# second-state/qwen3_asr_rs

Measured on AMD Instinct MI355X. Metric: audio-seconds/sec (RTFx) Qwen3-ASR-0.6B greedy, 30s clips, higher is better.
Workload: dtype bf16; 1 GPU; Qwen3-ASR-0.6b bf16, batch=1 x 30s synthetic 16kHz clip per GPU, 100 new tokens (fixed, EOS ignored); clips_per_gpu=1, parallelism=dp1 (independent utterances per GPU, no data-path collective)

## Files before the change

### qwen3_asr_rs_amd/csrc/dev.h

```cpp
#pragma once
#include <hip/hip_runtime.h>
#include <stdint.h>

#ifdef Q3A_STAMP
#define Q3A_STAMP_FIELD unsigned long long* stamp = nullptr;
#define Q3A_STAMP_AT(ptr, wg, slot) do { if ((ptr) && threadIdx.x == 0) (ptr)[(size_t)(wg) * 8 + (slot)] = wall_clock64(); } while (0)
#else
#define Q3A_STAMP_FIELD
#define Q3A_STAMP_AT(ptr, wg, slot) do { } while (0)
#endif

#define Q3A_ARG(x) asm volatile("" ::"s"(x))

namespace q3a {

typedef __attribute__((ext_vector_type(8))) __bf16 bf16x8_t;
typedef __attribute__((ext_vector_type(4))) float f32x4_t;
typedef __attribute__((ext_vector_type(2))) float f32x2_t;
typedef __attribute__((ext_vector_type(16))) float f32x16_t;

__device__ __forceinline__ float bf16_bits_to_f32(uint32_t v) { return __uint_as_float(v << 16); }
typedef __attribute__((ext_vector_type(2))) __bf16 bf16x2_t;
__device__ __forceinline__ uint32_t pack_bf16x2(float lo, float hi) {
  const f32x2_t v = {lo, hi};
// ... 105 lines not shown

__device__ __forceinline__ float lane_bcast(float v, int lane_uniform) {
  return __int_as_float(__builtin_amdgcn_readlane(__float_as_int(v), lane_uniform));
}

__device__ __forceinline__ float own_vgpr(float x) {
  asm volatile("" : "+v"(x));
  return x;
}
__device__ __forceinline__ void rope_rotate(float n1, float n2, float c, float sn, float& x1, float& x2) {
  const float a = sn * n2, b = sn * n1;
  x1 = __builtin_fmaf(c, n1, -a);
  x2 = __builtin_fmaf(c, n2, b);
}

__device__ __forceinline__ void head_norm_rope(float& x1, float& x2, const float* __restrict__ w, float eps,
                                               const float* __restrict__ cos_t, const float* __restrict__ sin_t,
                                               int pos, int lane) {
  const float ss = wave_sum_fast(x1 * x1 + x2 * x2);
  const float rstd = 1.0f / sqrtf(ss / 128.0f + eps);
  const float c = cos_t[(size_t)pos * 64 + lane], sn = sin_t[(size_t)pos * 64 + lane];
  const float n1 = (x1 * rstd) * w[lane], n2 = (x2 * rstd) * w[lane + 64];
  rope_rotate(n1, n2, c, sn, x1, x2);
}

template <typename T> struct KvIo;
template <> struct KvIo<float> {
  static __device__ __forceinline__ float load(const float* p) { return *p; }
  static __device__ __forceinline__ void store(float* p, float v) { *p = v; }
  static __device__ __forceinline__ float round(float v) { return v; }
};
template <> struct KvIo<uint16_t> {
  static __device__ __forceinline__ float load(const uint16_t* p) { return bf16_bits_to_f32(*p); }
  static __device__ __forceinline__ void store(uint16_t* p, float v) { *p = (uint16_t)f32_to_bf16_bits(v); }
  static __device__ __forceinline__ float round(float v) { return bf16_bits_to_f32(f32_to_bf16_bits(v)); }
};

}
// ... 1 lines not shown
```

### qwen3_asr_rs_amd/csrc/engine.cpp

```cpp
#include <hip/hip_runtime.h>

#include <sched.h>

#include <algorithm>
#include <atomic>
#include <chrono>
#include <cmath>
#include <cstdio>
#include <cstring>
#include <map>
#include <memory>
#include <mutex>
#include <string>
#include <thread>
#include <vector>

#include "../../include/q3asr.h"
#include "kernels.h"
#include "model.h"

using namespace q3a;

namespace {

// ... 77 lines not shown
}
namespace q3a {
struct KnobEntry { const char* key; const char* env; std::atomic<int> Knobs::*field; };
static const KnobEntry kKnobTable[] = {
    {"gemm256_min_tiles", "Q3A_GEMM256_MIN_TILES", &Knobs::gemm256_min_tiles},
    {"gemm256_persist", "Q3A_GEMM256_PERSIST", &Knobs::gemm256_persist},
    {"gemm256_group_m", "Q3A_GEMM256_GROUP_M", &Knobs::gemm256_group_m},
    {"dattn_batched_min_wgs", "Q3A_DATTN_BATCHED_MIN_WGS", &Knobs::dattn_batched_min_wgs},
    {"decode_group_size", "Q3A_DECODE_GROUP", &Knobs::decode_group_size},
    {"decode_parallel_groups", "Q3A_DECODE_PARALLEL", &Knobs::decode_parallel_groups},
    {"fuse_qkrope", "Q3A_FUSE_QKROPE", &Knobs::fuse_qkrope},
    {"skinny_q", "Q3A_SKINNY_Q", &Knobs::skinny_q},
    {"eos_run_ahead", "Q3A_EOS_RUN_AHEAD", &Knobs::eos_run_ahead},
    {"skinny_glu_hp3", "Q3A_SKINNY_GLU_HP3", &Knobs::skinny_glu_hp3},
    {"lm_head_prune", "Q3A_LM_HEAD_PRUNE", &Knobs::lm_head_prune},
    {"layer_taps", "Q3A_DEBUG_LAYER_TAPS", &Knobs::layer_taps},
    {"poison_attn_partials", nullptr, &Knobs::poison_attn_partials},
};
Knobs& knobs() {
  static Knobs k;
  static std::once_flag once;
  std::call_once(once, [] {
    for (const KnobEntry& t : kKnobTable)
      if (const char* e = t.env ? getenv(t.env) : nullptr) (k.*t.field).store(atoi(e));
  });
  return k;
}
}

struct q3a_engine {
// ... 693 lines not shown
  void run_prefill_layers() {
    const int H = d.hidden, I = d.inter, QD = d.q_dim(), QKV = d.qkv_dim();
    const bool sp = precise();
    KCHK(launch_embed(ids.as<int>(), total_P, wh(L.embed), H, kAudioPad, dec_x.as<float>(), stream));
    scatter_audio_rows();
    tap("dec_embed", dec_x.p, (size_t)total_P * H * 4);
    AttnArgs at{};
    at.q = dec_qkv.as<float>(); at.q_rs = QKV; at.kv_hs = (int64_t)max_ctx * 128; at.kv_rs = 128;
    at.o = dec_ctx.as<float>(); at.o_rs = QD; at.segs = dec_segs.as<AttnSeg>(); at.n_segs = B;
    at.max_len = *std::max_element(P.begin(), P.end()); at.n_kv_heads = d.n_kv;
    at.scale_div = sqrtf((float)d.head_dim);
    at.o16 = valu_attn() ? nullptr : dec_ctx.as<uint16_t>();
    if (!valu_attn()) { at.q16 = dec_q16.as<uint16_t>(); at.q_rs = QD; }
    const DevBuf& ctx_in = (valu_attn() && !sp) ? dec_ctx16 : dec_ctx;
    const bool qkv_bias = arena_flags & kFlagDecQkvBias, o_bias = arena_flags & kFlagDecOBias, mlp_bias = arena_flags & kFlagDecMlpBias;
    const bool fuse_rope = knobs().fuse_qkrope.load() != 0 && !valu_attn() && !precise() && d.head_dim == 128 && gemm256_eligible(total_P, QKV, H) && H % 64 == 0;
    const bool layer_taps = opts.debug_taps && knobs().layer_taps.load() != 0;
    for (int li = 0; li < d.dec_layers; ++li) {
      const DecLayerOff& l = L.dec[li];
      auto ltap = [&](const char* what, const void* ptr, size_t bytes) {
        if (!layer_taps) return;
        char name[32];
        snprintf(name, sizeof(name), "L%02d_%s", li, what);
        tap(name, ptr, bytes);
      };
      KCHK(launch_rmsnorm(dec_x.as<float>(), wf(l.in_ln), dec_ln.as<float>(), total_P, H, d.rms_eps, stream, act16(dec_ln)));
      ltap("ln1", dec_ln.p, (size_t)total_P * H * act_elem());
      RopeKvArgs rk{};
      rk.qkv = dec_qkv.as<float>(); rk.row_seq = row_seq.as<int>(); rk.row_pos = row_pos.as<int>();
      rk.q_norm = wf(l.q_norm); rk.k_norm = wf(l.k_norm); rk.eps = d.rms_eps;
      rk.cos_t = rope_cos.as<float>(); rk.sin_t = rope_sin.as<float>();
      rk.kcache = kc_layer(li); rk.vcache = vc_layer(li); rk.n_q = d.n_q; rk.n_kv = d.n_kv; rk.max_ctx = max_ctx;
      rk.q16 = valu_attn() ? nullptr : dec_q16.as<uint16_t>();
      if (fuse_rope) {
        KCHK(launch_gemm256_qkrope(dec_ln.as<uint16_t>(), H, wh(l.qkv_w), total_P, H, qkv_bias ? wf(l.qkv_b) : nullptr, rk, stream));
      } else {
        GemmEpilogue ep; ep.out = dec_qkv.as<float>(); ep.ldo = QKV; ep.bias = qkv_bias ? wf(l.qkv_b) : nullptr;
        act_gemm(dec_ln, H, wh(l.qkv_w), total_P, QKV, H, ep, false);
        KCHK(launch_qknorm_rope_kv(rk, total_P, kv_f32(), stream));
      }
      at.k = kc_layer(li); at.v = vc_layer(li);
      if (fuse_rope) {
        ltap("qkvs", dec_qkv.p, std::min((size_t)1024, (size_t)total_P) * QKV * 4);
      }
      if (!valu_attn()) ltap("q", dec_q16.p, (size_t)total_P * QD * 2);
      ltap("k", kc_layer(li), (size_t)B * d.n_kv * max_ctx * 128 * kv_elem());
      ltap("v", vc_layer(li), (size_t)B * d.n_kv * max_ctx * 128 * kv_elem());
      if (valu_attn()) {
        KCHK(launch_attn_prefill(at, d.n_q / d.n_kv, kv_f32(), stream));
        if (!sp) KCHK(launch_to_bf16(dec_ctx.as<float>(), dec_ctx16.as<uint16_t>(), (size_t)total_P * QD, stream));
// ... 1522 lines not shown
```

### qwen3_asr_rs_amd/csrc/k_fattn.hip

```cpp
#include <stdlib.h>

#include "dev.h"
#include "kernels.h"

namespace q3a {
namespace {

#ifndef Q3A_FATTN_XCD_REMAP
#define Q3A_FATTN_XCD_REMAP 1
#endif
__device__ __forceinline__ void fattn_block(int& bx, int& by, int& bz) {
  bx = blockIdx.x; by = blockIdx.y; bz = blockIdx.z;
#if Q3A_FATTN_XCD_REMAP
  const int gx = gridDim.x, gy = gridDim.y, total = gx * gy * (int)gridDim.z;
  const int lin = bx + gx * (by + gy * bz);
  const int xcd = lin & 7, loc = lin >> 3, q = total >> 3, r = total & 7;
  const int id = (xcd < r ? xcd * (q + 1) : r * (q + 1) + (xcd - r) * q) + loc;
  bx = id % gx;
  const int t = id / gx;
  by = t % gy;
  bz = t / gy;
#endif
}

// ... 421 lines not shown
      for (int r4 = 0; r4 < 4; ++r4) {
        const int d = dt * 32 + 8 * r4 + 4 * half;
        const float4 v = make_float4(oacc[dt][4 * r4] * inv, oacc[dt][4 * r4 + 1] * inv, oacc[dt][4 * r4 + 2] * inv, oacc[dt][4 * r4 + 3] * inv);
        if (a.o16) {
          uint2 pk;
          pk.x = pack_bf16x2(v.x, v.y);
          pk.y = pack_bf16x2(v.z, v.w);
          *reinterpret_cast<uint2*>(a.o16 + (size_t)(seg.q_row0 + qi) * a.o_rs + head * HD + d) = pk;
        } else {
          *reinterpret_cast<float4*>(orow + d) = v;
        }
      }
  }
}

template <int HD, int GROUP, bool CAUSAL>
void launch_dma(const AttnArgs& a, hipStream_t s) {
  constexpr int QT = 32 * (4 / GROUP);
  dim3 grid((a.max_len + QT - 1) / QT, a.n_kv_heads, a.n_segs);
  static const int ns = [] { const char* e = getenv("Q3A_FATTN_NS"); return e ? atoi(e) : 3; }();
  if (ns == 4) hipLaunchKernelGGL((fattn_dma_kernel<HD, GROUP, CAUSAL, 4>), grid, dim3(256), 0, s, a);
  else hipLaunchKernelGGL((fattn_dma_kernel<HD, GROUP, CAUSAL, 3>), grid, dim3(256), 0, s, a);
}
static bool fattn_dma_on() {
  static const bool on = [] { const char* e = getenv("Q3A_FATTN_DMA"); return !e || atoi(e) != 0; }();
  return on;
}

static bool fattn_dma_ok(const AttnArgs& a) {
  const auto al16 = [](const void* p) { return (reinterpret_cast<uintptr_t>(p) & 15) == 0; };
// ... 18 lines not shown
    else launch_f<64, 1, false, uint16_t>(a, s);
  } else {
    launch_f<64, 1, false, float>(a, s);
  }
  return nullptr;
}

const char* launch_fattn_prefill(const AttnArgs& a, int group, hipStream_t s) {
  if (a.n_segs <= 0) return nullptr;
  if (a.q_rs % 4 != 0 || a.o_rs % 4 != 0) return "fattn: row strides must be multiples of 4";
  if (a.q16 && a.q_rs % 8 != 0) return "fattn: bf16 q row stride must be a multiple of 8";
  static const int ks_wgs = [] { const char* e = getenv("Q3A_FATTN_KSPLIT_MAX_WGS"); return e ? atoi(e) : 128; }();
  const long wgs64 = (long)((a.max_len + 63) / 64) * a.n_kv_heads * a.n_segs;
  const bool dma = fattn_dma_ok(a);
  if (group == 1) { if (dma) launch_dma<128, 1, true>(a, s); else launch_f<128, 1, true, uint16_t>(a, s); }
  else if (group == 2 && wgs64 < ks_wgs) launch_f<128, 2, true, uint16_t, 2>(a, s);
  else if (group == 2) { if (dma) launch_dma<128, 2, true>(a, s); else launch_f<128, 2, true, uint16_t>(a, s); }
  else if (group == 4) { if (dma) launch_dma<128, 4, true>(a, s); else launch_f<128, 4, true, uint16_t>(a, s); }
  else return "fattn: GQA group must be 1, 2 or 4";
  return nullptr;
}

}
```

### qwen3_asr_rs_amd/csrc/k_gemm16.hip

```cpp
#include <stdlib.h>

#include <type_traits>

#include "argmax.h"

namespace q3a {
namespace {

typedef const void __attribute__((address_space(1)))* gptr_t;
typedef void __attribute__((address_space(3)))* lptr_t;

struct DenseA16 {
  const uint16_t* x;
  int lda;
  __device__ __forceinline__ void init_row(int m, int M, int& s0, int& s1, int& s2) const {
    s0 = m < M ? m : M - 1;
    s1 = s2 = 0;
  }
  __device__ __forceinline__ const uint16_t* row_ptr(int s0, int, int, int k0) const { return x + (size_t)s0 * lda + k0; }
};

struct ConvA16 {
  const uint16_t* x;
  const uint16_t* zero;
// ... 9 lines not shown
    const int tap = k0 / C, c0 = k0 - tap * C;
    const int kh = tap / 3, kw = tap - kh * 3;
    const int ih = oh * 2 - 1 + kh, iw = ow * 2 - 1 + kw;
    if (ih < 0 || ih >= H || iw < 0 || iw >= W) return zero;
    return x + (((size_t)img * H + ih) * W + iw) * C + c0;
  }
};

template <int BK> __device__ __forceinline__ int swz(int row) { return BK == 64 ? (row >> 1) & 7 : (row >> 2) & 3; }

template <int N> __device__ __forceinline__ void g16_wait_vm() {
  static_assert(N >= 0 && N < 64, "vmcnt value");
  asm volatile("s_waitcnt vmcnt(%0)" ::"n"(N) : "memory");
}

template <int BM, int BN, int BK, bool GLU, class ALoader, int NS = 2, bool LP = false>
__global__ __launch_bounds__(256) void gemm16_kernel(ALoader A, const uint16_t* __restrict__ Wt, int M, int N, int K,
                                                     GemmEpilogue ep) {
  constexpr int CPR = BK / 8;
  constexpr int RPI = 64 / CPR;
  constexpr int A_LOADS = BM / (4 * RPI) > 0 ? BM / (4 * RPI) : 1;
  constexpr int W_LOADS = BN / (4 * RPI) > 0 ? BN / (4 * RPI) : 1;
  constexpr bool A_PART = BM < 4 * RPI, W_PART = BN < 4 * RPI;
  constexpr int MI = BM / 32, NI = BN / 32;
  static_assert(MI >= 1 && NI >= 1 && (!GLU || NI >= 2), "tile shape");
  static_assert(NS == 2 || ((NS == 3 || NS == 4) && !A_PART && !W_PART), "stage count");
  constexpr int STAGE = (BM + BN) * BK;
  __shared__ __attribute__((aligned(16))) uint16_t lds[NS * STAGE];
  Q3A_STAMP_AT(ep.stamp, blockIdx.x, 0);

  const int tiles_m = (M + BM - 1) / BM, tiles_n = (N + BN - 1) / BN;
  const int nwg = tiles_m * tiles_n;
  int bid = blockIdx.x;
  {
    const int q = nwg / 8, r = nwg % 8, xcd = bid % 8, loc = bid / 8;
    bid = (xcd < r ? xcd * (q + 1) : r * (q + 1) + (xcd - r) * q) + loc;
  }
  const int tm = bid % tiles_m, tn = bid / tiles_m;
  const int m0 = tm * BM, n0 = tn * BN;
  const int tid = threadIdx.x, lane = tid & 63, wave = tid >> 6;
  const int wr = wave >> 1, wc = wave & 1;

  const int l_row = lane / CPR, l_chunk = lane % CPR;
  const bool a_on = !A_PART || wave * RPI < BM, w_on = !W_PART || wave * RPI < BN;
  int a_s0[A_LOADS], a_s1[A_LOADS], a_s2[A_LOADS], a_src_chunk[A_LOADS];
  const uint16_t* w_src[W_LOADS];
#pragma unroll
  for (int i = 0; i < A_LOADS; ++i) {
    const int row = (i * 4 + wave) * RPI + l_row;
    a_src_chunk[i] = l_chunk ^ swz<BK>(row);
    A.init_row(m0 + row, M, a_s0[i], a_s1[i], a_s2[i]);
  }
#pragma unroll
  for (int i = 0; i < W_LOADS; ++i) {
    const int row = (i * 4 + wave) * RPI + l_row;
    const int n = n0 + row;
    w_src[i] = Wt + (size_t)(n < N ? n : N - 1) * K + (l_chunk ^ swz<BK>(row)) * 8;
// ... 29 lines not shown
      for (int i = 0; i < MI; ++i) {
        const int mc = mrow[i] < M ? mrow[i] : M - 1;
#pragma unroll
        for (int j = 0; j < NI; ++j) ad[i][j] = *reinterpret_cast<const float4*>(ep.addend + (size_t)(mc % ep.addend_period) * ep.ldo + ncl[j]);
      }
    }
    if (ep.resid) {
#pragma unroll
      for (int i = 0; i < MI; ++i) {
        const int oc = orow[i] < 0 ? 0 : orow[i];
#pragma unroll
        for (int j = 0; j < NI; ++j) rs[i][j] = *reinterpret_cast<const float4*>(ep.resid + (size_t)oc * ep.ldo + ncl[j]);
      }
    }
  };
  const bool pre = !GLU && MI * NI <= 4 && vec && ep.rowmap == nullptr;
  if (pre) load_operands();

  const int frag_row = lane & 15, frag_kc = lane >> 4;
  const int KT = K / BK;
  auto issue_tile = [&](int kt, int buf) {
    const int k0 = kt * BK;
    if (a_on) {
#pragma unroll
      for (int i = 0; i < A_LOADS; ++i) {
        const int base = (i * 4 + wave) * RPI * BK;
        const uint16_t* ap = A.row_ptr(a_s0[i], a_s1[i], a_s2[i], k0) + a_src_chunk[i] * 8;
        __builtin_amdgcn_global_load_lds((gptr_t)ap, (lptr_t)(lds + buf * STAGE + base), 16, 0, 0);
      }
    }
    if (w_on) {
#pragma unroll
// ... 34 lines not shown
      for (int j = 0; j < NI; ++j) {
        const int row = wc * (BN / 2) + j * 16 + frag_row;
        bfrag[j] = *reinterpret_cast<const bf16x8_t*>(&ws[row * BK + (((ks * 4 + frag_kc) ^ swz<BK>(row)) * 8)]);
      }
#pragma unroll
      for (int i = 0; i < MI; ++i) {
        const int row = wr * (BM / 2) + i * 16 + frag_row;
        const bf16x8_t af = *reinterpret_cast<const bf16x8_t*>(&as[row * BK + (((ks * 4 + frag_kc) ^ swz<BK>(row)) * 8)]);
#pragma unroll
        for (int j = 0; j < NI; ++j) acc[i][j] = __builtin_amdgcn_mfma_f32_16x16x32_bf16(bfrag[j], af, acc[i][j], 0, 0, 0);
      }
    }
  }

  Q3A_STAMP_AT(ep.stamp, blockIdx.x, 2);
  if (ep.rowmap) {
#pragma unroll
    for (int i = 0; i < MI; ++i) orow[i] = ep.rowmap[orow[i]];
  }
  if (!GLU && vec) {
    if (!pre) load_operands();
    constexpr bool ARGMAX = BM == 32 && MI == 1;
    static_assert(!LP || ARGMAX, "the log-sum channel rides on the argmax partials");
    ArgmaxAcc<LP> best;
    float lv[LP ? NI : 1][4];
    if constexpr (LP) {
#pragma unroll
      for (int j = 0; j < NI; ++j) lv[j][0] = lv[j][1] = lv[j][2] = lv[j][3] = -INFINITY;
    }
#pragma unroll
// ... 350 lines not shown
  if (n == 0) return nullptr;
  size_t blocks = (n + 255) / 256;
  if (blocks > 4096) blocks = 4096;
  hipLaunchKernelGGL(from_bf16_kernel, dim3((unsigned)blocks), dim3(256), 0, s, x, y, n);
  return nullptr;
}

const char* launch_gemm16(const uint16_t* X, int lda, const uint16_t* W, int M, int N, int K, const GemmEpilogue& ep,
                          bool glu, hipStream_t s) {
  if (M <= 0) return nullptr;
  if (K % 32 != 0 || lda % 8 != 0) return "gemm16: K must be a multiple of 32 and lda of 8";
  if (K % 64 == 0 && !ep.part.val && gemm256_eligible(M, N, K)) return launch_gemm256(X, lda, W, M, N, K, ep, glu, s);
  return launch_gemm16_small(X, lda, W, M, N, K, ep, glu, s);
}

const char* launch_gemm16_small(const uint16_t* X, int lda, const uint16_t* W, int M, int N, int K, const GemmEpilogue& ep,
                                bool glu, hipStream_t s) {
  if (M <= 0) return nullptr;
  if (K % 32 != 0 || lda % 8 != 0) return "gemm16: K must be a multiple of 32 and lda of 8";
  if (glu && N % 32 != 0) return "gemm16: GLU needs N % 32 == 0";
  if (const char* e = argmax_partials_check(ep.part, (N + 63) / 64)) return e;
  if (ep.part.val && (M > 32 || glu || N % 4 != 0 || ep.ldo % 4 != 0 || K % 64 != 0 || ep.rowmap))
    return "gemm16: argmax partials need M <= 32, 4 | N, 4 | ldo, 64 | K and no row map";
  DenseA16 A{X, lda};
  static const bool ksplit_on = [] { const char* e = getenv("Q3A_GEMM16_KSPLIT"); return !e || atoi(e) != 0; }();
  if (ksplit_on && !glu && !ep.part.val && tiles_of(M, N, 32, 64) < 384 && K >= 512 && K % 128 == 0 && N % 4 == 0 && ep.ldo % 4 == 0) {
    const int tiles = ((M + 31) / 32) * ((N + 31) / 32);
    if (K % 256 == 0) hipLaunchKernelGGL((gemm16k_kernel<32, 256, DenseA16, 2>), dim3(tiles), dim3(256), 0, s, A, W, M, N, K, ep);
    else hipLaunchKernelGGL((gemm16k_kernel<32, 128, DenseA16, 4>), dim3(tiles), dim3(256), 0, s, A, W, M, N, K, ep);
    return nullptr;
  }
  static const bool force_bk32 = [] { const char* e = getenv("Q3A_GEMM16_BK32"); return e && atoi(e) != 0; }();
  if (K % 64 == 0 && !force_bk32) {
    if (glu) launch_sized16<64, true>(A, W, M, N, K, ep, s); else launch_sized16<64, false>(A, W, M, N, K, ep, s);
  } else {
    if (glu) launch_sized16<32, true>(A, W, M, N, K, ep, s); else launch_sized16<32, false>(A, W, M, N, K, ep, s);
  }
  return nullptr;
}

const char* launch_to_bf16(const float* x, uint16_t* y, size_t n, hipStream_t s) {
  if (n == 0) return nullptr;
  if (n % 4 != 0) return "to_bf16: n must be a multiple of 4";
  size_t blocks = (n / 4 + 255) / 256;
  if (blocks > 4096) blocks = 4096;
  hipLaunchKernelGGL(to_bf16_kernel, dim3((unsigned)blocks), dim3(256), 0, s, x, y, n / 4);
  return nullptr;
}

const char* launch_conv3x3s2_gemm16(const uint16_t* X, const uint16_t* zero_page, int imgs, int H, int Wd, int C,
                                    const uint16_t* Wt, int Cout, const GemmEpilogue& ep, hipStream_t s) {
  if (C % 32 != 0) return "conv gemm16: C must be a multiple of 32";
// ... 11 lines not shown
```

### qwen3_asr_rs_amd/csrc/k_mel.hip

```cpp
#include "dev.h"
#include "kernels.h"

namespace q3a {
namespace {

constexpr int N_FFT = 400, HOP = 160, N_FREQ = 201, DFT_COLS = 416, N_MELS = 128;
constexpr int FRAMES_PER_BLOCK = 32;
constexpr int SAMPLES_PER_BLOCK = (FRAMES_PER_BLOCK - 1) * HOP + N_FFT;
constexpr int P_STRIDE = 209;
constexpr int K_MEL = 202;

__device__ __forceinline__ unsigned float_key(float x) {
  unsigned u = __float_as_uint(x);
  return (u & 0x80000000u) ? ~u : (u | 0x80000000u);
}
__device__ __forceinline__ float key_float(unsigned k) {
  return __uint_as_float((k & 0x80000000u) ? (k & 0x7fffffffu) : ~k);
}

__global__ __launch_bounds__(256) void mel_kernel(MelBatch mb, const float* __restrict__ dft,
                                                  const float* __restrict__ filt_t) {
  __shared__ float s_lds[SAMPLES_PER_BLOCK + SAMPLES_PER_BLOCK / HOP + 8];
  __shared__ float p_lds[FRAMES_PER_BLOCK * P_STRIDE];
  const int b = blockIdx.y;
  const int F = mb.n_frames[b];
  const int f0 = blockIdx.x * FRAMES_PER_BLOCK;
  if (f0 >= F) return;
  const int64_t n = mb.n_samples[b];
  const int64_t Lp = (int64_t)F * HOP;
  const float* pcm = mb.pcm + mb.pcm_off[b];
  const int tid = threadIdx.x, lane = tid & 63, wave = tid >> 6, half = lane >> 5, l31 = lane & 31;

  for (int p = tid; p < SAMPLES_PER_BLOCK; p += 256) {
    int64_t i = (int64_t)f0 * HOP + p - N_FFT / 2;
    if (i < 0) i = -i;
    else if (i >= Lp) i = 2 * (Lp - 1) - i;
    float v = 0.f;
    if (i >= 0 && i < n) v = pcm[i];
    s_lds[p + p / HOP] = v;
  }
  for (int i = tid; i < FRAMES_PER_BLOCK * P_STRIDE; i += 256) p_lds[i] = 0.f;
  __syncthreads();

  const int a_base = l31 * (HOP + 1);
  for (int tile = wave; tile < DFT_COLS / 32; tile += 4) {
    f32x16_t acc;
#pragma unroll
    for (int r = 0; r < 16; ++r) acc[r] = 0.f;
    const float* bcol = dft + tile * 32 + l31;
#pragma unroll 4
    for (int nn = 0; nn < N_FFT; nn += 2) {
      const int m = nn + half;
      const float a = s_lds[a_base + m + (m >= HOP) + (m >= 2 * HOP)];
      const float bv = bcol[(size_t)m * DFT_COLS];
      acc = __builtin_amdgcn_mfma_f32_32x32x2f32(a, bv, acc, 0, 0, 0);
    }
    const int c = tile * 32 + l31, k = c >> 1;
#pragma unroll
    for (int r = 0; r < 16; ++r) {
      float pw = acc[r] * acc[r];
      pw += __shfl_xor(pw, 1, 64);
      const int frame = (r & 3) + 8 * (r >> 2) + 4 * half;
      if ((c & 1) == 0 && k < P_STRIDE - 1) p_lds[frame * P_STRIDE + k] = pw;
    }
  }
  __syncthreads();

  f32x16_t acc;
#pragma unroll
  for (int r = 0; r < 16; ++r) acc[r] = 0.f;
  const float* acol = filt_t + wave * 32 + l31;
  const float* brow = p_lds + l31 * P_STRIDE;
#pragma unroll 4
  for (int kk = 0; kk < K_MEL; kk += 2) {
    const int k = kk + half;
    acc = __builtin_amdgcn_mfma_f32_32x32x2f32(acol[(size_t)k * N_MELS], brow[k], acc, 0, 0, 0);
  }
  const int f = f0 + l31;
  float vmax = -3.0e38f;
  float* out = mb.mel + mb.mel_off[b];
#pragma unroll
  for (int r = 0; r < 16; ++r) {
    const int m = wave * 32 + (r & 3) + 8 * (r >> 2) + 4 * half;
    const float lv = log10f(fmaxf(acc[r], 1e-10f));
    if (f < F) {
      out[(size_t)m * F + f] = lv;
      vmax = fmaxf(vmax, lv);
    }
  }
  vmax = wave_max(vmax);
  if (lane == 0) atomicMax(mb.gmax_key + b, float_key(vmax));
// ... 4 lines not shown
  const int64_t total = (int64_t)mb.n_frames[b] * N_MELS;
  const float floor_v = key_float(mb.gmax_key[b]) - 8.0f;
  float* m = mb.mel + mb.mel_off[b];
  for (int64_t i = (int64_t)blockIdx.x * blockDim.x + threadIdx.x; i < total; i += (int64_t)gridDim.x * blockDim.x)
    m[i] = (fmaxf(m[i], floor_v) + 4.0f) / 4.0f;
}

}

const char* launch_mel(const MelBatch& mb, int B, int max_frames, const float* dft, const float* filt_t,
                       hipStream_t s) {
  if (B <= 0) return nullptr;
  hipError_t e = hipMemsetAsync(mb.gmax_key, 0, sizeof(unsigned) * B, s);
  if (e != hipSuccess) return "mel: memset failed";
  const int tiles = (max_frames + FRAMES_PER_BLOCK - 1) / FRAMES_PER_BLOCK;
  hipLaunchKernelGGL(mel_kernel, dim3(tiles, B), dim3(256), 0, s, mb, dft, filt_t);
  int fb = (max_frames * N_MELS + 255) / 256;
  if (fb > 1024) fb = 1024;
  hipLaunchKernelGGL(mel_finalize_kernel, dim3(fb, B), dim3(256), 0, s, mb);
  return nullptr;
}

}
```

### qwen3_asr_rs_amd/csrc/kernels.h

```cpp
#pragma once
#include <hip/hip_runtime.h>
#include <stdint.h>

#include <atomic>

#ifndef Q3A_STAMP_FIELD
#ifdef Q3A_STAMP
#define Q3A_STAMP_FIELD unsigned long long* stamp = nullptr;
#else
#define Q3A_STAMP_FIELD
#endif
#endif

namespace q3a {

struct ArgmaxPartials {
  float* val = nullptr;
  int* idx = nullptr;
  float* sum = nullptr;
  int stride = 0;
  ArgmaxPartials at(size_t rows) const {
    const size_t o = rows * stride;
    return {val ? val + o : nullptr, idx ? idx + o : nullptr, sum ? sum + o : nullptr, stride};
  }
// ... 63 lines not shown
bool gemm256_eligible(int M, int N, int K);
const char* launch_gemm16_small(const uint16_t* X, int lda, const uint16_t* W, int M, int N, int K, const GemmEpilogue& ep,
                                bool glu, hipStream_t s);
struct Knobs {
  std::atomic<int> gemm256_min_tiles{128};
  std::atomic<int> gemm256_persist{1};
  std::atomic<int> gemm256_group_m{0};
  std::atomic<int> dattn_batched_min_wgs{128};
  std::atomic<int> decode_group_size{0};
  std::atomic<int> decode_parallel_groups{1};
  std::atomic<int> fuse_qkrope{1};
  std::atomic<int> skinny_q{1};
  std::atomic<int> eos_run_ahead{1};
  std::atomic<int> skinny_glu_hp3{1};
  std::atomic<int> lm_head_prune{1};
  std::atomic<int> layer_taps{0};
  std::atomic<int> poison_attn_partials{0};
};
Knobs& knobs();
const char* launch_gemm256(const uint16_t* X, int lda, const uint16_t* W, int M, int N, int K, const GemmEpilogue& ep,
                           bool glu, hipStream_t s);
const char* launch_conv3x3s2_gemm256(const uint16_t* X, const uint16_t* zero_page, int imgs, int H, int Wd, int C,
                                     const uint16_t* Wt, int Cout, const GemmEpilogue& ep, hipStream_t s);
const char* launch_to_bf16(const float* x, uint16_t* y, size_t n, hipStream_t s);
const char* launch_from_bf16(const uint16_t* x, float* y, size_t n, hipStream_t s);

struct MelBatch {
  const float* pcm;
  const int64_t* pcm_off;
  const int64_t* n_samples;
// ... 41 lines not shown
const char* launch_embed(const int* ids, int rows, const uint16_t* embed, int H, int skip_id, float* out, hipStream_t s);
struct RopeKvArgs {
  float* qkv;
  const int* row_seq;
  const int* row_pos;
  const float* q_norm; const float* k_norm; float eps;
  const float* cos_t; const float* sin_t;
  void* kcache; void* vcache;
  int n_q, n_kv, max_ctx;
  uint16_t* q16;
};
const char* launch_qknorm_rope_kv(const RopeKvArgs& a, int rows, bool kv_f32, hipStream_t s);
int gemm256_split_rows(int M, int N);
const char* launch_gemm256_qkrope(const uint16_t* X, int lda, const uint16_t* W, int M, int K, const float* bias,
                                  const RopeKvArgs& a, hipStream_t s);
const char* launch_gather_rows(const float* src, const int* row_idx, int n, int D, float* dst, hipStream_t s);
const char* launch_scatter_rows(const float* src, const int* dst_row, int n, int D, float* dst, hipStream_t s);

struct GemvArgs {
  const float* x; int ldx;
  const float* rms_w;
  float eps;
  const uint16_t* W; int N; int K;
  const float* bias;
  int mode;
  float* out; int ldo;
  const float* resid;
  ArgmaxPartials part;
  const float* attn_pm; const float* attn_pl; const float* attn_po; int attn_nsplit; int attn_heads;
  int attn_fast_exp;
// ... 150 lines not shown
```

Baseline: 483.6 audio-seconds/sec.

## Add gemm16 QK-norm/RoPE fused epilogue, key-split DMA attention, and mel DFT prefetch

Three separate changes land together. First, a QK-norm+RoPE+KV-write epilogue is fused into the small gemm16 kernel, so prefill shapes that miss gemm256 no longer run a separate rope kernel. Second, a new flash-attention kernel for GQA group 2 splits the keys across two wave pairs, streams K/V into LDS through a global_load_lds ring, and merges the two halves at the end. Third, the mel kernel register-prefetches DFT and filterbank operands in groups to overlap loads with MFMA. All three add code paths and register or LDS pressure, and each sits behind a knob that is on by default.

After: 482.1 audio-seconds/sec. No clear change (-0.3%).

```diff
diff --git a/qwen3_asr_rs_amd/csrc/dev.h b/qwen3_asr_rs_amd/csrc/dev.h
--- a/qwen3_asr_rs_amd/csrc/dev.h
+++ b/qwen3_asr_rs_amd/csrc/dev.h
@@ -143,14 +143,16 @@
   x2 = __builtin_fmaf(c, n2, b);
 }
 
+__device__ __forceinline__ void head_norm_rope_cs(float& x1, float& x2, float w1, float w2, float eps, float c, float sn) {
+  const float ss = wave_sum_fast(x1 * x1 + x2 * x2);
+  const float rstd = 1.0f / sqrtf(ss / 128.0f + eps);
+  const float n1 = (x1 * rstd) * w1, n2 = (x2 * rstd) * w2;
+  rope_rotate(n1, n2, c, sn, x1, x2);
+}
 __device__ __forceinline__ void head_norm_rope(float& x1, float& x2, const float* __restrict__ w, float eps,
                                                const float* __restrict__ cos_t, const float* __restrict__ sin_t,
                                                int pos, int lane) {
-  const float ss = wave_sum_fast(x1 * x1 + x2 * x2);
-  const float rstd = 1.0f / sqrtf(ss / 128.0f + eps);
-  const float c = cos_t[(size_t)pos * 64 + lane], sn = sin_t[(size_t)pos * 64 + lane];
-  const float n1 = (x1 * rstd) * w[lane], n2 = (x2 * rstd) * w[lane + 64];
-  rope_rotate(n1, n2, c, sn, x1, x2);
+  head_norm_rope_cs(x1, x2, w[lane], w[lane + 64], eps, cos_t[(size_t)pos * 64 + lane], sin_t[(size_t)pos * 64 + lane]);
 }
 
 template <typename T> struct KvIo;
diff --git a/qwen3_asr_rs_amd/csrc/engine.cpp b/qwen3_asr_rs_amd/csrc/engine.cpp
--- a/qwen3_asr_rs_amd/csrc/engine.cpp
+++ b/qwen3_asr_rs_amd/csrc/engine.cpp
@@ -115,6 +115,8 @@
     {"eos_run_ahead", "Q3A_EOS_RUN_AHEAD", &Knobs::eos_run_ahead},
     {"skinny_glu_hp3", "Q3A_SKINNY_GLU_HP3", &Knobs::skinny_glu_hp3},
     {"lm_head_prune", "Q3A_LM_HEAD_PRUNE", &Knobs::lm_head_prune},
+    {"fattn_ksplit_dma", "Q3A_FATTN_KSPLIT_DMA", &Knobs::fattn_ksplit_dma},
+    {"mel_prefetch", "Q3A_MEL_PREFETCH", &Knobs::mel_prefetch},
     {"layer_taps", "Q3A_DEBUG_LAYER_TAPS", &Knobs::layer_taps},
     {"poison_attn_partials", nullptr, &Knobs::poison_attn_partials},
 };
@@ -838,7 +840,9 @@
     if (!valu_attn()) { at.q16 = dec_q16.as<uint16_t>(); at.q_rs = QD; }
     const DevBuf& ctx_in = (valu_attn() && !sp) ? dec_ctx16 : dec_ctx;
     const bool qkv_bias = arena_flags & kFlagDecQkvBias, o_bias = arena_flags & kFlagDecOBias, mlp_bias = arena_flags & kFlagDecMlpBias;
-    const bool fuse_rope = knobs().fuse_qkrope.load() != 0 && !valu_attn() && !precise() && d.head_dim == 128 && gemm256_eligible(total_P, QKV, H) && H % 64 == 0;
+    const bool fuse_ok = knobs().fuse_qkrope.load() != 0 && !valu_attn() && !precise() && d.head_dim == 128;
+    const bool fuse_rope = fuse_ok && gemm256_eligible(total_P, QKV, H) && H % 64 == 0;
+    const bool fuse_rope16 = fuse_ok && !fuse_rope && gemm16_qkrope_eligible(total_P, QKV, H);
     const bool layer_taps = opts.debug_taps && knobs().layer_taps.load() != 0;
     for (int li = 0; li < d.dec_layers; ++li) {
       const DecLayerOff& l = L.dec[li];
@@ -858,6 +862,8 @@
       rk.q16 = valu_attn() ? nullptr : dec_q16.as<uint16_t>();
       if (fuse_rope) {
         KCHK(launch_gemm256_qkrope(dec_ln.as<uint16_t>(), H, wh(l.qkv_w), total_P, H, qkv_bias ? wf(l.qkv_b) : nullptr, rk, stream));
+      } else if (fuse_rope16) {
+        KCHK(launch_gemm16_qkrope(dec_ln.as<uint16_t>(), H, wh(l.qkv_w), total_P, H, qkv_bias ? wf(l.qkv_b) : nullptr, rk, stream));
       } else {
         GemmEpilogue ep; ep.out = dec_qkv.as<float>(); ep.ldo = QKV; ep.bias = qkv_bias ? wf(l.qkv_b) : nullptr;
         act_gemm(dec_ln, H, wh(l.qkv_w), total_P, QKV, H, ep, false);
diff --git a/qwen3_asr_rs_amd/csrc/k_fattn.hip b/qwen3_asr_rs_amd/csrc/k_fattn.hip
--- a/qwen3_asr_rs_amd/csrc/k_fattn.hip
+++ b/qwen3_asr_rs_amd/csrc/k_fattn.hip
@@ -459,6 +459,233 @@
   }
 }
 
+template <int HD, int GROUP, bool CAUSAL, int NS>
+__global__ __launch_bounds__(256) void fattn_ksplit_dma_kernel(AttnArgs a) {
+  static_assert(GROUP == 2, "4 waves = 2 key halves x 2 query heads");
+  constexpr int KT = 64;
+  constexpr int KS = HD / 16, DT = HD / 32;
+  constexpr int ROW_B = HD * 2;
+  constexpr int RPP = 1024 / ROW_B;
+  constexpr int CPR = HD / 8;
+  constexpr int PIECES = KT / RPP;
+  constexpr int PPW = PIECES / 4;
+  constexpr int OPB = KT * ROW_B;
+  constexpr int STAGE = 2 * OPB;
+  constexpr int MERGE_B = GROUP * (32 * HD + 64) * 4;
+  static_assert(PPW >= 1 && NS * STAGE >= MERGE_B, "ring shape");
+  __shared__ __attribute__((aligned(1024))) uint8_t ring[NS * STAGE];
+
+  int blk_x, blk_y, blk_z;
+  fattn_block(blk_x, blk_y, blk_z);
+  const AttnSeg seg = a.segs[blk_z];
+  const int kvh = blk_y;
+  const int qb0 = blk_x * 32;
+  if (qb0 >= seg.len) return;
+  const int tid = threadIdx.x, lane = tid & 63;
+  const int wave = __builtin_amdgcn_readfirstlane(tid >> 6);
+  const int l31 = lane & 31, half = lane >> 5;
+  const int g = wave % GROUP, kh = wave / GROUP;
+  const int head = kvh * GROUP + g;
+  const int q0 = qb0, qi = q0 + l31;
+  const uint16_t* kbase = reinterpret_cast<const uint16_t*>(a.k) + seg.kv_off + (int64_t)kvh * a.kv_hs;
+  const uint16_t* vbase = reinterpret_cast<const uint16_t*>(a.v) + seg.kv_off + (int64_t)kvh * a.kv_hs;
+
+  const int block_qmax = min(qb0 + 32, seg.len) - 1;
+  const int n_keys = CAUSAL ? block_qmax + 1 : seg.len;
+  const int n_tiles = (n_keys + KT - 1) / KT;
+  const int wave_qmax = block_qmax;
+
+  const int prow = lane / CPR, pc = lane % CPR;
+  int srcK[PPW], srcV[PPW], rowt[PPW];
+#pragma unroll
+  for (int i = 0; i < PPW; ++i) {
+    const int p = wave * PPW + i, r = p * RPP + prow;
+    rowt[i] = r;
+    srcK[i] = HD == 128 ? (pc ^ (r & 15)) : (pc ^ ((r >> 1) & 7));
+    const int b = pc >> 1, bs = HD == 128 ? (b ^ (2 * (r & 3))) : (b ^ (r & 2));
+    srcV[i] = (bs << 1) | (pc & 1);
+  }
+  const int last_key = seg.len - 1;
+  auto issue = [&](int t) {
+    uint8_t* st = ring + (t % NS) * STAGE;
+#pragma unroll
+    for (int i = 0; i < PPW; ++i) {
+      const int key = min(t * KT + rowt[i], last_key);
+      const int p = wave * PPW + i;
+      __builtin_amdgcn_global_load_lds((fa_gptr_t)(kbase + (int64_t)key * a.kv_rs + srcK[i] * 8), (fa_lptr_t)(st + p * 1024), 16, 0, 0);
+      __builtin_amdgcn_global_load_lds((fa_gptr_t)(vbase + (int64_t)key * a.kv_rs + srcV[i] * 8), (fa_lptr_t)(st + OPB + p * 1024), 16, 0, 0);
+    }
+  };
+  constexpr int PER_TILE = 2 * PPW;
+#pragma unroll
+  for (int t = 0; t < NS - 1; ++t)
+    if (t < n_tiles) issue(t);
+
+  bf16x8_t qfrag[KS];
+  {
+    const uint16_t* qrow = a.q16 + (size_t)(seg.q_row0 + (qi < seg.len ? qi : seg.len - 1)) * a.q_rs + head * HD;
+#pragma unroll
+    for (int ks = 0; ks < KS; ++ks) qfrag[ks] = *reinterpret_cast<const bf16x8_t*>(qrow + ks * 16 + half * 8);
+#pragma unroll
+    for (int ks = 0; ks < KS; ++ks) asm volatile("" : "+v"(qfrag[ks]));
+  }
+
+  f32x16_t oacc[DT];
+#pragma unroll
+  for (int dt = 0; dt < DT; ++dt)
+#pragma unroll
+    for (int r = 0; r < 16; ++r) oacc[dt][r] = 0.f;
+  float mrun = -INFINITY, lrun = 0.f;
+  const float inv_scale = 1.0f / a.scale_div;
+
+  int koff[KS];
+#pragma unroll
+  for (int ks = 0; ks < KS; ++ks) {
+    const int c = ks * 2 + half;
+    koff[ks] = (kh * 32 + l31) * ROW_B + ((HD == 128 ? (c ^ (l31 & 15)) : (c ^ ((l31 >> 1) & 7))) << 4);
+  }
+  const int vr = (lane & 15) >> 2, vu = lane & 3, db = (lane >> 4) & 1;
+  unsigned voff[DT];
+#pragma unroll
+  for (int dt = 0; dt < DT; ++dt) {
+    const int b = dt * 2 + db, bs = HD == 128 ? (b ^ (2 * vr)) : (b ^ (vr & 2));
+    voff[dt] = (kh * 32 + 4 * half + vr) * ROW_B + bs * 32 + vu * 8;
+  }
+
+  for (int t = 0; t < n_tiles; ++t) {
+    const int later = min(NS - 2, n_tiles - 1 - t);
+    if (NS >= 4 && later >= 2) asm volatile("s_waitcnt vmcnt(%0)" ::"n"(2 * PER_TILE) : "memory");
+    else if (later >= 1) asm volatile("s_waitcnt vmcnt(%0)" ::"n"(PER_TILE) : "memory");
+    else asm volatile("s_waitcnt vmcnt(0)" ::: "memory");
+    asm volatile("s_barrier" ::: "memory");
+    if (t + NS - 1 < n_tiles) issue(t + NS - 1);
+    const uint8_t* st = ring + (t % NS) * STAGE;
+    const int key0 = t * KT + kh * 32;
+    if (CAUSAL && key0 > wave_qmax) continue;
+
+    f32x16_t sacc;
+#pragma unroll
+    for (int r = 0; r < 16; ++r) sacc[r] = 0.f;
+#pragma unroll
+    for (int ks = 0; ks < KS; ++ks) {
+      const bf16x8_t kf = *reinterpret_cast<const bf16x8_t*>(st + koff[ks]);
+      sacc = __builtin_amdgcn_mfma_f32_32x32x16_bf16(kf, qfrag[ks], sacc, 0, 0, 0);
+    }
+    const bool full = key0 + 31 <= (CAUSAL ? min(q0, seg.len - 1) : seg.len - 1);
+    float tmax = -INFINITY;
+    if (full) {
+#pragma unroll
+      for (int r = 0; r < 16; ++r) {
+        sacc[r] *= inv_scale;
+        tmax = fmaxf(tmax, sacc[r]);
+      }
+    } else {
+#pragma unroll
+      for (int r = 0; r < 16; ++r) {
+        const int key = key0 + (r & 3) + 8 * (r >> 2) + 4 * half;
+        const bool valid = key < seg.len && (!CAUSAL || key <= qi);
+        sacc[r] = valid ? sacc[r] * inv_scale : -INFINITY;
+        tmax = fmaxf(tmax, sacc[r]);
+      }
+    }
+    tmax = xor32_max(tmax);
+    const float m_new = fmaxf(mrun, tmax);
+    const bool rescale = __builtin_amdgcn_ballot_w64(m_new > mrun) != 0;
+    float alpha = 1.f, psum = 0.f;
+    if (m_new == -INFINITY) {
+#pragma unroll
+      for (int r = 0; r < 16; ++r) sacc[r] = 0.f;
+    } else {
+      alpha = __expf(mrun - m_new);
+#pragma unroll
+      for (int r = 0; r < 16; ++r) {
+        sacc[r] = __expf(sacc[r] - m_new);
+        psum += sacc[r];
+      }
+    }
+    psum = xor32_sum(psum);
+    lrun = lrun * alpha + psum;
+    mrun = m_new;
+    bf16x8_t pfrag[2];
+#pragma unroll
+    for (int kk = 0; kk < 2; ++kk) {
+      uint4 p;
+      p.x = pack_bf16x2(sacc[kk * 8 + 0], sacc[kk * 8 + 1]); p.y = pack_bf16x2(sacc[kk * 8 + 2], sacc[kk * 8 + 3]);
+      p.z = pack_bf16x2(sacc[kk * 8 + 4], sacc[kk * 8 + 5]); p.w = pack_bf16x2(sacc[kk * 8 + 6], sacc[kk * 8 + 7]);
+      pfrag[kk] = *reinterpret_cast<const bf16x8_t*>(&p);
+    }
+    const unsigned vstage = (unsigned)(size_t)(st + OPB);
+    typedef unsigned fa_u2 __attribute__((ext_vector_type(2)));
+    fa_u2 vt[DT][4];
+    auto tr_reads = [&](int dt) {
+      const unsigned ad = vstage + voff[dt];
+      asm volatile("ds_read_b64_tr_b16 %0, %1" : "=v"(vt[dt][0]) : "v"(ad) : "memory");
+      asm volatile("ds_read_b64_tr_b16 %0, %1 offset:%2" : "=v"(vt[dt][1]) : "v"(ad), "n"(8 * ROW_B) : "memory");
+      asm volatile("ds_read_b64_tr_b16 %0, %1 offset:%2" : "=v"(vt[dt][2]) : "v"(ad), "n"(16 * ROW_B) : "memory");
+      asm volatile("ds_read_b64_tr_b16 %0, %1 offset:%2" : "=v"(vt[dt][3]) : "v"(ad), "n"(24 * ROW_B) : "memory");
+    };
+    tr_reads(0);
+#pragma unroll
+    for (int dt = 0; dt < DT; ++dt) {
+      if (rescale) {
+        asm volatile("" ::: "memory");
+        oacc[dt] *= alpha;
+      }
+      if (dt + 1 < DT) {
+        tr_reads(dt + 1);
+        asm volatile("s_waitcnt lgkmcnt(4)" : "+v"(vt[dt][0]), "+v"(vt[dt][1]), "+v"(vt[dt][2]), "+v"(vt[dt][3])::"memory");
+      } else {
+        asm volatile("s_waitcnt lgkmcnt(0)" : "+v"(vt[dt][0]), "+v"(vt[dt][1]), "+v"(vt[dt][2]), "+v"(vt[dt][3])::"memory");
+      }
+#pragma unroll
+      for (int kk = 0; kk < 2; ++kk) {
+        const uint4 v = make_uint4(vt[dt][kk * 2].x, vt[dt][kk * 2].y, vt[dt][kk * 2 + 1].x, vt[dt][kk * 2 + 1].y);
+        oacc[dt] = __builtin_amdgcn_mfma_f32_32x32x16_bf16(__builtin_bit_cast(bf16x8_t, v), pfrag[kk], oacc[dt], 0, 0, 0);
+      }
+    }
+  }
+  __syncthreads();
+  float* const mo = reinterpret_cast<float*>(ring) + g * (32 * HD + 64);
+  if (kh == 1) {
+#pragma unroll
+    for (int dt = 0; dt < DT; ++dt)
+#pragma unroll
+      for (int r = 0; r < 16; ++r) mo[(dt * 16 + r) * 64 + lane] = oacc[dt][r];
+    if (half == 0) { mo[32 * HD + l31] = mrun; mo[32 * HD + 32 + l31] = lrun; }
+  }
+  __syncthreads();
+  if (kh == 1) return;
+  const float m2 = mo[32 * HD + l31], l2 = mo[32 * HD + 32 + l31];
+  const float mn = fmaxf(mrun, m2);
+  if (mn != -INFINITY) {
+    const float f1 = __expf(mrun - mn), f2 = __expf(m2 - mn);
+    lrun = lrun * f1 + l2 * f2;
+#pragma unroll
+    for (int dt = 0; dt < DT; ++dt)
+#pragma unroll
+      for (int r = 0; r < 16; ++r) oacc[dt][r] = oacc[dt][r] * f1 + mo[(dt * 16 + r) * 64 + lane] * f2;
+  }
+  if (qi < seg.len) {
+    const float inv = 1.0f / lrun;
+    float* orow = a.o + (size_t)(seg.q_row0 + qi) * a.o_rs + head * HD;
+#pragma unroll
+    for (int dt = 0; dt < DT; ++dt)
+#pragma unroll
+      for (int r4 = 0; r4 < 4; ++r4) {
+        const int d = dt * 32 + 8 * r4 + 4 * half;
+        const float4 v = make_float4(oacc[dt][4 * r4] * inv, oacc[dt][4 * r4 + 1] * inv, oacc[dt][4 * r4 + 2] * inv, oacc[dt][4 * r4 + 3] * inv);
+        if (a.o16) {
+          uint2 pk;
+          pk.x = pack_bf16x2(v.x, v.y);
+          pk.y = pack_bf16x2(v.z, v.w);
+          *reinterpret_cast<uint2*>(a.o16 + (size_t)(seg.q_row0 + qi) * a.o_rs + head * HD + d) = pk;
+        } else {
+          *reinterpret_cast<float4*>(orow + d) = v;
+        }
+      }
+  }
+}
+
 template <int HD, int GROUP, bool CAUSAL>
 void launch_dma(const AttnArgs& a, hipStream_t s) {
   constexpr int QT = 32 * (4 / GROUP);
@@ -507,7 +734,14 @@
   const long wgs64 = (long)((a.max_len + 63) / 64) * a.n_kv_heads * a.n_segs;
   const bool dma = fattn_dma_ok(a);
   if (group == 1) { if (dma) launch_dma<128, 1, true>(a, s); else launch_f<128, 1, true, uint16_t>(a, s); }
-  else if (group == 2 && wgs64 < ks_wgs) launch_f<128, 2, true, uint16_t, 2>(a, s);
+  else if (group == 2 && wgs64 < ks_wgs) {
+    if (dma && knobs().fattn_ksplit_dma.load() != 0) {
+      dim3 grid((a.max_len + 31) / 32, a.n_kv_heads, a.n_segs);
+      hipLaunchKernelGGL((fattn_ksplit_dma_kernel<128, 2, true, 3>), grid, dim3(256), 0, s, a);
+    } else {
+      launch_f<128, 2, true, uint16_t, 2>(a, s);
+    }
+  }
   else if (group == 2) { if (dma) launch_dma<128, 2, true>(a, s); else launch_f<128, 2, true, uint16_t>(a, s); }
   else if (group == 4) { if (dma) launch_dma<128, 4, true>(a, s); else launch_f<128, 4, true, uint16_t>(a, s); }
   else return "fattn: GQA group must be 1, 2 or 4";
diff --git a/qwen3_asr_rs_amd/csrc/k_gemm16.hip b/qwen3_asr_rs_amd/csrc/k_gemm16.hip
--- a/qwen3_asr_rs_amd/csrc/k_gemm16.hip
+++ b/qwen3_asr_rs_amd/csrc/k_gemm16.hip
@@ -47,9 +47,15 @@
   asm volatile("s_waitcnt vmcnt(%0)" ::"n"(N) : "memory");
 }
 
-template <int BM, int BN, int BK, bool GLU, class ALoader, int NS = 2, bool LP = false>
+struct NoRope {};
+struct RopeEp { RopeKvArgs a; };
+
+template <int BM, int BN, int BK, bool GLU, class ALoader, int NS = 2, bool LP = false, class Rope = NoRope>
 __global__ __launch_bounds__(256) void gemm16_kernel(ALoader A, const uint16_t* __restrict__ Wt, int M, int N, int K,
-                                                     GemmEpilogue ep) {
+                                                     GemmEpilogue ep, Rope rope = Rope{}) {
+  constexpr bool ROPE = std::is_same<Rope, RopeEp>::value;
+  static_assert(!ROPE || (BN == 128 && !GLU && !LP && BM % 4 == 0), "the rope epilogue takes one 128-wide head per column tile");
+  constexpr int RPW = ROPE ? BM / 4 : 1;
   constexpr int CPR = BK / 8;
   constexpr int RPI = 64 / CPR;
   constexpr int A_LOADS = BM / (4 * RPI) > 0 ? BM / (4 * RPI) : 1;
@@ -74,6 +80,17 @@
   const int tid = threadIdx.x, lane = tid & 63, wave = tid >> 6;
   const int wr = wave >> 1, wc = wave & 1;
 
+  int r_pos[RPW], r_seq[RPW];
+  float r_cos[RPW], r_sin[RPW], r_w1 = 0.f, r_w2 = 0.f;
+  if constexpr (ROPE) {
+#pragma unroll
+    for (int rr = 0; rr < RPW; ++rr) {
+      const int row = m0 + wave * RPW + rr < M ? m0 + wave * RPW + rr : M - 1;
+      r_pos[rr] = rope.a.row_pos[row];
+      r_seq[rr] = rope.a.row_seq[row];
+    }
+  }
+
   const int l_row = lane / CPR, l_chunk = lane % CPR;
   const bool a_on = !A_PART || wave * RPI < BM, w_on = !W_PART || wave * RPI < BN;
   int a_s0[A_LOADS], a_s1[A_LOADS], a_s2[A_LOADS], a_src_chunk[A_LOADS];
@@ -133,8 +150,19 @@
       }
     }
   };
-  const bool pre = !GLU && MI * NI <= 4 && vec && ep.rowmap == nullptr;
+  const bool pre = ROPE || (!GLU && MI * NI <= 4 && vec && ep.rowmap == nullptr);
   if (pre) load_operands();
+  if constexpr (ROPE) {
+    if (tn < rope.a.n_q + rope.a.n_kv) {
+      const float* w = tn < rope.a.n_q ? rope.a.q_norm : rope.a.k_norm;
+      r_w1 = w[lane]; r_w2 = w[lane + 64];
+#pragma unroll
+      for (int rr = 0; rr < RPW; ++rr) {
+        r_cos[rr] = rope.a.cos_t[(size_t)r_pos[rr] * 64 + lane];
+        r_sin[rr] = rope.a.sin_t[(size_t)r_pos[rr] * 64 + lane];
+      }
+    }
+  }
 
   const int frag_row = lane & 15, frag_kc = lane >> 4;
   const int KT = K / BK;
@@ -199,6 +227,50 @@
   }
 
   Q3A_STAMP_AT(ep.stamp, blockIdx.x, 2);
+  if constexpr (ROPE) {
+    constexpr int SP = BN + 4;
+    static_assert(NS * STAGE * 2 >= BM * SP * 4, "the staged tile must fit in the stages");
+    const RopeKvArgs& a = rope.a;
+    float* st = reinterpret_cast<float*>(lds);
+    __syncthreads();
+#pragma unroll
+    for (int i = 0; i < MI; ++i)
+#pragma unroll
+      for (int j = 0; j < NI; ++j) {
+        float v[4] = {acc[i][j][0], acc[i][j][1], acc[i][j][2], acc[i][j][3]};
+        if (ep.bias) { v[0] += bb[j].x; v[1] += bb[j].y; v[2] += bb[j].z; v[3] += bb[j].w; }
+        *reinterpret_cast<float4*>(&st[(wr * (BM / 2) + i * 16 + m_in) * SP + wc * (BN / 2) + j * 16 + n_in]) = make_float4(v[0], v[1], v[2], v[3]);
+      }
+    __syncthreads();
+    const int hv = tn, nvec = a.n_q + 2 * a.n_kv;
+#pragma unroll
+    for (int rr = 0; rr < RPW; ++rr) {
+      const int row = m0 + wave * RPW + rr;
+      if (row >= M) break;
+      float x1 = st[(wave * RPW + rr) * SP + lane], x2 = st[(wave * RPW + rr) * SP + lane + 64];
+      if (hv < a.n_q) {
+        head_norm_rope_cs(x1, x2, r_w1, r_w2, a.eps, r_cos[rr], r_sin[rr]);
+        if (a.q16) {
+          uint16_t* q = a.q16 + (size_t)row * a.n_q * 128 + (size_t)hv * 128;
+          q[lane] = (uint16_t)f32_to_bf16_bits(x1);
+          q[lane + 64] = (uint16_t)f32_to_bf16_bits(x2);
+        } else {
+          float* base = a.qkv + (size_t)row * nvec * 128 + (size_t)hv * 128;
+          base[lane] = x1;
+          base[lane + 64] = x2;
+        }
+      } else {
+        const bool is_k = hv < a.n_q + a.n_kv;
+        const int kvh = is_k ? hv - a.n_q : hv - a.n_q - a.n_kv;
+        if (is_k) head_norm_rope_cs(x1, x2, r_w1, r_w2, a.eps, r_cos[rr], r_sin[rr]);
+        uint16_t* c = reinterpret_cast<uint16_t*>(is_k ? a.kcache : a.vcache) + (((size_t)r_seq[rr] * a.n_kv + kvh) * a.max_ctx + r_pos[rr]) * 128;
+        KvIo<uint16_t>::store(c + lane, x1);
+        KvIo<uint16_t>::store(c + lane + 64, x2);
+      }
+    }
+    Q3A_STAMP_AT(ep.stamp, blockIdx.x, 3);
+    return;
+  }
   if (ep.rowmap) {
 #pragma unroll
     for (int i = 0; i < MI; ++i) orow[i] = ep.rowmap[orow[i]];
@@ -579,6 +651,12 @@
   return launch_gemm16_small(X, lda, W, M, N, K, ep, glu, s);
 }
 
+static bool gemm16_ksplit_on() {
+  static const bool on = [] { const char* e = getenv("Q3A_GEMM16_KSPLIT"); return !e || atoi(e) != 0; }();
+  return on;
+}
+static bool ksplit_shape(int M, int N, int K, int ldo);
+
 const char* launch_gemm16_small(const uint16_t* X, int lda, const uint16_t* W, int M, int N, int K, const GemmEpilogue& ep,
                                 bool glu, hipStream_t s) {
   if (M <= 0) return nullptr;
@@ -588,8 +666,7 @@
   if (ep.part.val && (M > 32 || glu || N % 4 != 0 || ep.ldo % 4 != 0 || K % 64 != 0 || ep.rowmap))
     return "gemm16: argmax partials need M <= 32, 4 | N, 4 | ldo, 64 | K and no row map";
   DenseA16 A{X, lda};
-  static const bool ksplit_on = [] { const char* e = getenv("Q3A_GEMM16_KSPLIT"); return !e || atoi(e) != 0; }();
-  if (ksplit_on && !glu && !ep.part.val && tiles_of(M, N, 32, 64) < 384 && K >= 512 && K % 128 == 0 && N % 4 == 0 && ep.ldo % 4 == 0) {
+  if (gemm16_ksplit_on() && !glu && !ep.part.val && ksplit_shape(M, N, K, ep.ldo)) {
     const int tiles = ((M + 31) / 32) * ((N + 31) / 32);
     if (K % 256 == 0) hipLaunchKernelGGL((gemm16k_kernel<32, 256, DenseA16, 2>), dim3(tiles), dim3(256), 0, s, A, W, M, N, K, ep);
     else hipLaunchKernelGGL((gemm16k_kernel<32, 128, DenseA16, 4>), dim3(tiles), dim3(256), 0, s, A, W, M, N, K, ep);
@@ -601,6 +678,30 @@
   } else {
     if (glu) launch_sized16<32, true>(A, W, M, N, K, ep, s); else launch_sized16<32, false>(A, W, M, N, K, ep, s);
   }
+  return nullptr;
+}
+
+static bool ksplit_shape(int M, int N, int K, int ldo) {
+  return tiles_of(M, N, 32, 64) < 384 && K >= 512 && K % 128 == 0 && N % 4 == 0 && ldo % 4 == 0;
+}
+
+bool gemm16_qkrope_eligible(int M, int N, int K) {
+  return K % 64 == 0 && N % 128 == 0 && !gemm256_eligible(M, N, K) && !(gemm16_ksplit_on() && ksplit_shape(M, N, K, N));
+}
+
+const char* launch_gemm16_qkrope(const uint16_t* X, int lda, const uint16_t* W, int M, int K, const float* bias,
+                                 const RopeKvArgs& rk, hipStream_t s) {
+  if (M <= 0) return nullptr;
+  const int N = (rk.n_q + 2 * rk.n_kv) * 128;
+  if (K % 64 != 0 || lda % 8 != 0) return "gemm16 qkrope: K must be a multiple of 64 and lda of 8";
+  if ((!rk.q16 && !rk.qkv) || !rk.kcache || !rk.vcache || !rk.row_pos || !rk.row_seq) return "gemm16 qkrope: q output / bf16 KV cache / row tables required";
+  GemmEpilogue ep;
+  ep.bias = bias; ep.ldo = N;
+  DenseA16 A{X, lda};
+  RopeEp rope{rk};
+  const int tiles = ((M + 31) / 32) * (N / 128);
+  if (tiles <= 256) hipLaunchKernelGGL((gemm16_kernel<32, 128, 64, false, DenseA16, 4, false, RopeEp>), dim3(tiles), dim3(256), 0, s, A, W, M, N, K, ep, rope);
+  else hipLaunchKernelGGL((gemm16_kernel<32, 128, 64, false, DenseA16, 3, false, RopeEp>), dim3(tiles), dim3(256), 0, s, A, W, M, N, K, ep, rope);
   return nullptr;
 }
 
diff --git a/qwen3_asr_rs_amd/csrc/k_mel.hip b/qwen3_asr_rs_amd/csrc/k_mel.hip
--- a/qwen3_asr_rs_amd/csrc/k_mel.hip
+++ b/qwen3_asr_rs_amd/csrc/k_mel.hip
@@ -18,6 +18,26 @@
   return __uint_as_float((k & 0x80000000u) ? (k & 0x7fffffffu) : ~k);
 }
 
+constexpr int DFT_GROUP = 25;
+constexpr int DFT_GROUPS = N_FFT / 2 / DFT_GROUP;
+constexpr int MEL_STEPS = K_MEL / 2;
+static_assert(DFT_GROUPS * DFT_GROUP * 2 == N_FFT && DFT_GROUPS % 2 == 0, "DFT groups come in pairs");
+
+__device__ __forceinline__ void mel_load_group(float (&buf)[DFT_GROUP], const float* __restrict__ bcol, int g, int half) {
+#pragma unroll
+  for (int i = 0; i < DFT_GROUP; ++i) buf[i] = bcol[(size_t)((g * DFT_GROUP + i) * 2 + half) * DFT_COLS];
+}
+__device__ __forceinline__ void mel_mfma_group(f32x16_t& acc, const float (&buf)[DFT_GROUP], const float* s_lds, int a_base, int g,
+                                               int half) {
+#pragma unroll
+  for (int i = 0; i < DFT_GROUP; ++i) {
+    const int m = (g * DFT_GROUP + i) * 2 + half;
+    const float a = s_lds[a_base + m + (m >= HOP) + (m >= 2 * HOP)];
+    acc = __builtin_amdgcn_mfma_f32_32x32x2f32(a, buf[i], acc, 0, 0, 0);
+  }
+}
+
+template <bool PF>
 __global__ __launch_bounds__(256) void mel_kernel(MelBatch mb, const float* __restrict__ dft,
                                                   const float* __restrict__ filt_t) {
   __shared__ float s_lds[SAMPLES_PER_BLOCK + SAMPLES_PER_BLOCK / HOP + 8];
@@ -29,7 +49,16 @@
   const int64_t n = mb.n_samples[b];
   const int64_t Lp = (int64_t)F * HOP;
   const float* pcm = mb.pcm + mb.pcm_off[b];
-  const int tid = threadIdx.x, lane = tid & 63, wave = tid >> 6, half = lane >> 5, l31 = lane & 31;
+  const int tid = threadIdx.x, lane = tid & 63, half = lane >> 5, l31 = lane & 31;
+  const int wave = PF ? __builtin_amdgcn_readfirstlane(tid >> 6) : tid >> 6;
+
+  const float* acol = filt_t + wave * 32 + l31;
+  float b0[PF ? DFT_GROUP : 1], b1[PF ? DFT_GROUP : 1], fa[PF ? MEL_STEPS : 1];
+  if constexpr (PF) {
+#pragma unroll
+    for (int i = 0; i < MEL_STEPS; ++i) fa[i] = acol[(size_t)(2 * i + half) * N_MELS];
+    mel_load_group(b0, dft + wave * 32 + l31, 0, half);
+  }
 
   for (int p = tid; p < SAMPLES_PER_BLOCK; p += 256) {
     int64_t i = (int64_t)f0 * HOP + p - N_FFT / 2;
@@ -43,17 +72,30 @@
   __syncthreads();
 
   const int a_base = l31 * (HOP + 1);
+#pragma unroll 1
   for (int tile = wave; tile < DFT_COLS / 32; tile += 4) {
     f32x16_t acc;
 #pragma unroll
     for (int r = 0; r < 16; ++r) acc[r] = 0.f;
     const float* bcol = dft + tile * 32 + l31;
+    if constexpr (PF) {
+      const float* bnext = tile + 4 < DFT_COLS / 32 ? bcol + 4 * 32 : bcol;
+#pragma unroll 1
+      for (int g = 0; g < DFT_GROUPS; g += 2) {
+        mel_load_group(b1, bcol, g + 1, half);
+        mel_mfma_group(acc, b0, s_lds, a_base, g, half);
+        const bool more = g + 2 < DFT_GROUPS;
+        mel_load_group(b0, more ? bcol : bnext, more ? g + 2 : 0, half);
+        mel_mfma_group(acc, b1, s_lds, a_base, g + 1, half);
+      }
+    } else {
 #pragma unroll 4
-    for (int nn = 0; nn < N_FFT; nn += 2) {
-      const int m = nn + half;
-      const float a = s_lds[a_base + m + (m >= HOP) + (m >= 2 * HOP)];
-      const float bv = bcol[(size_t)m * DFT_COLS];
-      acc = __builtin_amdgcn_mfma_f32_32x32x2f32(a, bv, acc, 0, 0, 0);
+      for (int nn = 0; nn < N_FFT; nn += 2) {
+        const int m = nn + half;
+        const float a = s_lds[a_base + m + (m >= HOP) + (m >= 2 * HOP)];
+        const float bv = bcol[(size_t)m * DFT_COLS];
+        acc = __builtin_amdgcn_mfma_f32_32x32x2f32(a, bv, acc, 0, 0, 0);
+      }
     }
     const int c = tile * 32 + l31, k = c >> 1;
 #pragma unroll
@@ -69,12 +111,16 @@
   f32x16_t acc;
 #pragma unroll
   for (int r = 0; r < 16; ++r) acc[r] = 0.f;
-  const float* acol = filt_t + wave * 32 + l31;
   const float* brow = p_lds + l31 * P_STRIDE;
+  if constexpr (PF) {
+#pragma unroll
+    for (int i = 0; i < MEL_STEPS; ++i) acc = __builtin_amdgcn_mfma_f32_32x32x2f32(fa[i], brow[2 * i + half], acc, 0, 0, 0);
+  } else {
 #pragma unroll 4
-  for (int kk = 0; kk < K_MEL; kk += 2) {
-    const int k = kk + half;
-    acc = __builtin_amdgcn_mfma_f32_32x32x2f32(acol[(size_t)k * N_MELS], brow[k], acc, 0, 0, 0);
+    for (int kk = 0; kk < K_MEL; kk += 2) {
+      const int k = kk + half;
+      acc = __builtin_amdgcn_mfma_f32_32x32x2f32(acol[(size_t)k * N_MELS], brow[k], acc, 0, 0, 0);
+    }
   }
   const int f = f0 + l31;
   float vmax = -3.0e38f;
@@ -109,7 +155,8 @@
   hipError_t e = hipMemsetAsync(mb.gmax_key, 0, sizeof(unsigned) * B, s);
   if (e != hipSuccess) return "mel: memset failed";
   const int tiles = (max_frames + FRAMES_PER_BLOCK - 1) / FRAMES_PER_BLOCK;
-  hipLaunchKernelGGL(mel_kernel, dim3(tiles, B), dim3(256), 0, s, mb, dft, filt_t);
+  if (knobs().mel_prefetch.load() != 0) hipLaunchKernelGGL((mel_kernel<true>), dim3(tiles, B), dim3(256), 0, s, mb, dft, filt_t);
+  else hipLaunchKernelGGL((mel_kernel<false>), dim3(tiles, B), dim3(256), 0, s, mb, dft, filt_t);
   int fb = (max_frames * N_MELS + 255) / 256;
   if (fb > 1024) fb = 1024;
   hipLaunchKernelGGL(mel_finalize_kernel, dim3(fb, B), dim3(256), 0, s, mb);
diff --git a/qwen3_asr_rs_amd/csrc/kernels.h b/qwen3_asr_rs_amd/csrc/kernels.h
--- a/qwen3_asr_rs_amd/csrc/kernels.h
+++ b/qwen3_asr_rs_amd/csrc/kernels.h
@@ -101,6 +101,8 @@
   std::atomic<int> eos_run_ahead{1};
   std::atomic<int> skinny_glu_hp3{1};
   std::atomic<int> lm_head_prune{1};
+  std::atomic<int> fattn_ksplit_dma{1};
+  std::atomic<int> mel_prefetch{1};
   std::atomic<int> layer_taps{0};
   std::atomic<int> poison_attn_partials{0};
 };
@@ -172,6 +174,9 @@
 int gemm256_split_rows(int M, int N);
 const char* launch_gemm256_qkrope(const uint16_t* X, int lda, const uint16_t* W, int M, int K, const float* bias,
                                   const RopeKvArgs& a, hipStream_t s);
+bool gemm16_qkrope_eligible(int M, int N, int K);
+const char* launch_gemm16_qkrope(const uint16_t* X, int lda, const uint16_t* W, int M, int K, const float* bias,
+                                 const RopeKvArgs& a, hipStream_t s);
 const char* launch_gather_rows(const float* src, const int* row_idx, int n, int D, float* dst, hipStream_t s);
 const char* launch_scatter_rows(const float* src, const int* dst_row, int n, int D, float* dst, hipStream_t s);
 
```
